# fuenshu/deap

Hardware: AMD Instinct MI355X
Metric: individual-generations/sec @pop=2^20 Rastrigin-1000D, 1-8 GPU; % HBM peak (higher is better)
Workload: dtype f64; 1 GPU; C3 Rastrigin-1000D fp64 eaSimple; pop_per_island=1048576, islands=1, islands_per_gpu=1, genes=1000, operators=selTournament(t=3) cxBlend mutGaussian cxpb=0.5 mutpb=0.2 indpb=0.05, parallelism=islands1

## Files before the change

deap_amd/csrc/capi.hip:

```cpp
#include <stdarg.h>
#include <stdio.h>

#include "common.hpp"
#include "evals.hpp"

namespace dm {

int zig_make_tables(double* t) {
    const double R = 3.6541528853610088, V = 0.00492867323399;
    double* x = t;
    double* f = t + (ZIG_N + 1);
    x[0] = V / std::exp(-0.5 * R * R);
    x[1] = R;
    for (int i = 2; i < ZIG_N; ++i)
        x[i] = std::sqrt(-2.0 * std::log(V / x[i - 1] + std::exp(-0.5 * x[i - 1] * x[i - 1])));
    x[ZIG_N] = 0.0;
    for (int i = 0; i <= ZIG_N; ++i) f[i] = std::exp(-0.5 * x[i] * x[i]);
    return DM_OK;
}

static thread_local char g_err[1024] = "";

void set_error(const char* fmt, ...) {
    va_list ap;
// ... 391 lines not shown
using namespace dm;

extern "C" {

const char* dm_last_error(void) { return dm::g_err; }
const char* dm_version(void) { return "deapmi 0.1 gfx950"; }

static int env_int(const char* name, int dflt) {
    const char* v = std::getenv(name);
    return v ? atoi(v) : dflt;
}

static void read_knobs(dm_knobs& kn) {
    kn.disable_pipe = std::getenv("DM_DISABLE_PIPE") != nullptr;
    kn.bits_plan = std::getenv("DM_BITS_PLAN") != nullptr;
    kn.bits_nokeys = std::getenv("DM_BITS_NOKEYS") != nullptr;
    kn.lex_full = std::getenv("DM_LEX_FULL") != nullptr;
    kn.lex_no32 = std::getenv("DM_LEX_NO32") != nullptr;
    kn.pipe_label_rounds = std::max(0, std::min(8, env_int("DM_PIPE_LABEL_ROUNDS", 2)));
    kn.selbest_fullsort = std::getenv("DM_SELBEST_FULLSORT") != nullptr;
    kn.pipe_bpc = std::max(0, env_int("DM_PIPE_BPC", 0));
    kn.pipe_noorder = std::getenv("DM_PIPE_NOORDER") != nullptr;
    kn.pipe_key_fitter = std::getenv("DM_PIPE_KEY_FITTER") != nullptr;
}

int dm_ctx_reload_knobs(dm_ctx* ctx) {
    DM_CHECK_ARG(ctx != nullptr, "null ctx");
    read_knobs(ctx->knobs);
    return DM_OK;
}

int dm_ctx_create(int device, void* hip_stream, dm_ctx** out) {
    DM_CHECK_ARG(out != nullptr, "null out");
    DM_HIP(hipSetDevice(device));
    dm_ctx* c = new dm_ctx();
    c->device = device;
    c->stream = (hipStream_t)hip_stream;
    read_knobs(c->knobs);
    int cus = 0;
    if (hipDeviceGetAttribute(&cus, hipDeviceAttributeMultiprocessorCount, device) == hipSuccess &&
        cus > 0)
        c->num_cus = cus;
    double tab[2 * (ZIG_N + 1)];
    zig_make_tables(tab);
    if (hipMalloc(&c->zig, sizeof(tab)) != hipSuccess ||
        hipMemcpy(c->zig, tab, sizeof(tab), hipMemcpyHostToDevice) != hipSuccess) {
// ... 279 lines not shown
```

deap_amd/csrc/common.hpp:

```cpp
#pragma once
#include <hip/hip_runtime.h>
#include <stdint.h>

#include <algorithm>
#include <cmath>
#include <cstdlib>
#include <string>
#include <vector>

#include "../../include/deapmi.h"

namespace dm {

void set_error(const char* fmt, ...);

#define DM_CHECK_ARG(cond, ...)                 \
    do {                                        \
        if (!(cond)) {                          \
            ::dm::set_error(__VA_ARGS__);       \
            return DM_ERR_INVALID;              \
        }                                       \
    } while (0)

#define DM_HIP(expr)                                                          \
// ... 3 lines not shown
            ::dm::set_error("HIP error %s at %s:%d: %s", hipGetErrorName(e_), \
                            __FILE__, __LINE__, #expr);                       \
            return DM_ERR_HIP;                                                \
        }                                                                     \
    } while (0)

#define DM_LAUNCH_CHECK() DM_HIP(hipGetLastError())

}

constexpr int kEvalSpread = 64, kEvalSpreadStride = 16;
constexpr int kEvalSpreadWords = (2 * kEvalSpread + 2) * kEvalSpreadStride;
struct dm_knobs {
    bool disable_pipe = false;
    bool bits_plan = false;
    bool bits_nokeys = false;
    bool lex_full = false;
    bool lex_no32 = false;
    int32_t pipe_label_rounds = 2;
    bool selbest_fullsort = false;
    int pipe_bpc = 0;
    bool pipe_noorder = false;
    bool pipe_key_fitter = false;
};

struct dm_ctx {
    static constexpr int kSlots = 5;
    int device = 0;
    hipStream_t stream = nullptr;
    void* scratch[kSlots] = {nullptr, nullptr, nullptr, nullptr, nullptr};
    size_t scratch_bytes[kSlots] = {0, 0, 0, 0, 0};
    void* pinned = nullptr;
    size_t pinned_bytes = 0;
    int num_cus = 256;
    int peel_hint = 4;
    int peel_trend = 0;
    int64_t peel_hint_U = 0, peel_hint_N = 0;
    double* zig = nullptr;
    long long* evals_spread = nullptr;
    std::vector<hipEvent_t> tev;
    int tev_used = 0;
    int timing_target = 0;
    dm_knobs knobs;
    uint64_t* plan_lab = nullptr;
    int64_t plan_lab_n = 0;
    uint32_t plan_epoch = 0;
// ... 183 lines not shown
```

deap_amd/csrc/generation.hip:

```cpp
#include "generation_pipe.hpp"
#include "sort.hpp"

namespace dm {

__global__ __launch_bounds__(256) void zero2_kernel(int32_t* __restrict__ a, int32_t* __restrict__ b,
                                                    int64_t n) {
    const int64_t n4 = n >> 2;
    const int64_t step = (int64_t)gridDim.x * blockDim.x;
    for (int64_t i = (int64_t)blockIdx.x * blockDim.x + threadIdx.x; i < n4; i += step) {
        reinterpret_cast<int4*>(a)[i] = make_int4(0, 0, 0, 0);
        if (b) reinterpret_cast<int4*>(b)[i] = make_int4(0, 0, 0, 0);
    }
    for (int64_t i = 4 * n4 + (int64_t)blockIdx.x * blockDim.x + threadIdx.x; i < n; i += step) {
        a[i] = 0;
        if (b) b[i] = 0;
    }
}

static int pick_group_float(int dim) {
    const int q = (dim + 3) / 4;
    if (q <= 4) return 4;
    if (q <= 16) return 16;
    return 64;
}
// ... 104 lines not shown
    a.sigma = var->sigma;
    a.mu_vec = var->mu_vec;
    a.sigma_vec = var->sigma_vec;
    a.flip_inv_log2 = (var->indpb > 0.0 && var->indpb < 1.0)
                          ? (float)(1.0 / std::log2(1.0 - var->indpb))
                          : 0.0f;
    a.eval_fn = ev->fn;
    a.w0 = ev->weights[0];
    a.ev = *ev;
    a.rng = Rng(rng);
    a.zig = ctx->zig;
    a.mode = mode;
    a.dec = d;
    a.nevals = nevals;

    const int ec = eval_class(ev->fn);
    const int64_t npairs = (children->n + 1) / 2;
    if (mode == DM_RNG_NATIVE && parents->gtype != DM_BITS && parents->dim > 64 &&
        parents->dim <= 65535 && (sel == DM_SEL_TOURNAMENT || sel == DM_SEL_RANDOM) &&
        ec != EC_MO && !ctx->knobs.disable_pipe) {
        const int nch = parents->dim <= 512 ? 2 : parents->dim <= 1024 ? 4 : 0;
        const bool ordered = !ctx->knobs.pipe_noorder && npairs >= 4096 &&
                             npairs < (1ll << (32 - PF_PAIR_SHIFT));
        const size_t pb = align_up((size_t)npairs * sizeof(PairPlan), 256);
        const size_t hb = align_up((size_t)(a.np + 1) * 4, 256);
        const size_t kb = align_up((size_t)npairs * 4, 256);
        char* w = (char*)scratch(ctx, ordered ? 2 * pb + 3 * hb + 4 * kb +
                                                    align_up(scan_temp_bytes(a.np), 256) : pb);
        if (!w) return DM_ERR_NOMEM;
        PairPlan* plans = (PairPlan*)w;
        const bool count = ec != EC_NONE && a.nevals;
        if (ordered) {
            PairPlan* sorted = (PairPlan*)(w + pb);
            int32_t* hist = (int32_t*)(w + 2 * pb);
            int32_t* start = (int32_t*)(w + 2 * pb + hb);
            int32_t* keys = (int32_t*)(w + 2 * pb + 2 * hb);
            int32_t* tick = (int32_t*)(w + 2 * pb + 2 * hb + kb);
            void* stemp = w + 2 * pb + 2 * hb + 2 * kb;
            const unsigned zg = (unsigned)std::min<int64_t>(2048, (a.np / 4 + 255) / 256 + 1);
            if (!ctx->knobs.pipe_key_fitter && ctx->knobs.pipe_label_rounds > 0) {
                uint32_t epoch = 0;
                uint64_t* lab64 = plan_labels(ctx, a.np, &epoch);
                if (!lab64) return DM_ERR_NOMEM;
                int2* pairs2 = (int2*)((char*)stemp + align_up(scan_temp_bytes(a.np), 256));
                launch_pair_plans(a, plans, count ? ctx->evals_spread : nullptr, ctx->stream,
                                  nullptr, nullptr, nullptr, lab64, epoch, pairs2, hist, a.np + 1);
                const int rounds = ctx->knobs.pipe_label_rounds;
                if (rounds > 2)
                    launch_plan_labels(pairs2, lab64, epoch, npairs, rounds - 2, ctx->stream);
                launch_plan_degree_keys(plans, pairs2, nullptr, lab64, epoch, rounds >= 2, keys,
                                        tick, hist, npairs, ctx->stream);
            } else if (!ctx->knobs.pipe_key_fitter) {
                int32_t* deg = (int32_t*)((char*)stemp + align_up(scan_temp_bytes(a.np), 256));
                zero2_kernel<<<zg, 256, 0, ctx->stream>>>(hist, deg, a.np);
                launch_pair_plans(a, plans, count ? ctx->evals_spread : nullptr, ctx->stream,
                                  nullptr, deg);
                launch_plan_degree_keys(plans, nullptr, deg, nullptr, 0, false, keys, tick, hist,
                                        npairs, ctx->stream);
            } else {
                zero2_kernel<<<zg, 256, 0, ctx->stream>>>(hist, nullptr, a.np);
                launch_pair_plans(a, plans, count ? ctx->evals_spread : nullptr, ctx->stream, keys,
                                  hist, tick);
            }
            int rc = exclusive_scan_i32(ctx->stream, hist, start, a.np, nullptr, stemp);
            if (rc) return rc;
            launch_plan_order(plans, keys, tick, start, sorted, npairs, ctx->stream);
            plans = sorted;
        } else {
            launch_pair_plans(a, plans, count ? ctx->evals_spread : nullptr, ctx->stream);
        }
        DM_LAUNCH_CHECK();
        PipeArgs q{};
        q.pgenes = a.pgenes;
        q.cgenes = a.cgenes;
        q.cwv = a.cwv;
        q.cvalid = a.cvalid;
        q.plans = plans;
        q.pwv = a.pwv;
        q.mu_vec = a.mu_vec;
        q.sigma_vec = a.sigma_vec;
        q.zig = a.zig;
        q.nevals = nullptr;
        q.nc = a.nc;
        q.pstride = a.pstride;
        q.cstride = a.cstride;
        q.dim = a.dim;
        q.nobj = a.nobj;
        q.rng = a.rng;
        q.thr_ind = a.thr_ind;
        q.alpha = a.alpha;
        q.mu = a.mu;
        q.sigma = a.sigma;
        q.w0 = a.w0;
        q.ev = a.ev;
        q.bpc = ctx->knobs.pipe_bpc;
        q.ordered = ordered ? 1 : 0;
        timing_begin(ctx);
        if (parents->gtype == DM_F64)
            launch_gen_pipe_f64(q, ec, a.cx, a.mut, nch, ctx->num_cus, ctx->stream);
        else
            launch_gen_pipe_f32(q, ec, a.cx, a.mut, nch, ctx->num_cus, ctx->stream);
        timing_end(ctx);
        DM_LAUNCH_CHECK();
        return DM_OK;
    }
    if (mode == DM_RNG_NATIVE && parents->gtype != DM_BITS && parents->dim <= 64 &&
        (sel == DM_SEL_TOURNAMENT || sel == DM_SEL_RANDOM) && !ctx->knobs.disable_pipe) {
        PairPlan* plans = (PairPlan*)scratch(ctx, align_up((size_t)npairs * sizeof(PairPlan), 256));
        if (!plans) return DM_ERR_NOMEM;
        const bool count = ec != EC_NONE && a.nevals;
        launch_pair_plans(a, plans, count ? ctx->evals_spread : nullptr, ctx->stream);
        DM_LAUNCH_CHECK();
        timing_begin(ctx);
        if (parents->gtype == DM_F64)
            launch_gen_rows_f64(a, plans, ec, ctx->num_cus, ctx->stream);
        else
            launch_gen_rows_f32(a, plans, ec, ctx->num_cus, ctx->stream);
        timing_end(ctx);
        DM_LAUNCH_CHECK();
// ... 64 lines not shown
```

deap_amd/csrc/generation_pipe.hpp:

```cpp
#pragma once
#include "generation.hpp"

namespace dm {

typedef __attribute__((address_space(4))) const uint32_t c4_u32;

#ifndef DM_RAST_ILP
#define DM_RAST_ILP 2
#endif

struct PairPlan {
    int32_t s0, s1;
    uint32_t cuts;
    uint32_t flags;
    double f0, f1;
};
static_assert(sizeof(PairPlan) == 32, "PairPlan layout");
enum : uint32_t { PF_CX = 1, PF_MUT0 = 2, PF_MUT1 = 4, PF_HAS1 = 8, PF_INV0 = 16, PF_INV1 = 32 };
constexpr int PF_PAIR_SHIFT = 8;

__device__ __forceinline__ PairPlan load_plan(const PairPlan* plans, int64_t p) {
    const c4_u32* q = (const c4_u32*)(const void*)(plans + p);
    uint32_t v[8];
#pragma unroll
    for (int i = 0; i < 8; ++i) v[i] = q[i];
    PairPlan r;
    r.s0 = (int32_t)v[0];
    r.s1 = (int32_t)v[1];
    r.cuts = v[2];
    r.flags = v[3];
    r.f0 = __hiloint2double((int)v[5], (int)v[4]);
    r.f1 = __hiloint2double((int)v[7], (int)v[6]);
    return r;
}

#ifndef DM_ZIG_SLOW_NOINLINE
#define DM_ZIG_SLOW_NOINLINE 1
#endif
#if DM_ZIG_SLOW_NOINLINE
__device__ __noinline__
#else
__device__ __forceinline__
// ... 141 lines not shown
                const double v = k == 0 ? x[0] : k == 1 ? x[1] : k == 2 ? x[2] : x[3];
                if (L::gene(c, lane, k) < dim) t += sum_term(ev.fn, v);
            }
            acc += t;
        }
    }
}

struct PipeArgs {
    const char* pgenes;
    char* cgenes;
    double* cwv;
    uint8_t* cvalid;
    const PairPlan* plans;
    const double* pwv;
    const double* mu_vec;
    const double* sigma_vec;
    const double* zig;
    int64_t* nevals;
    int64_t nc, pstride, cstride;
    int32_t dim, nobj;
    int32_t bpc;
    int32_t ordered;
    Rng rng;
    uint64_t thr_ind;
    double alpha, mu, sigma, w0;
    dm_eval ev;
};

#ifndef DM_PIPE_MINWAVES
#define DM_PIPE_MINWAVES 2
#endif

#ifndef DM_PIPE_ABLATE
#define DM_PIPE_ABLATE 0
#endif

#ifndef DM_PIPE_DEPTH
#define DM_PIPE_DEPTH 2
#endif

template <typename T, int NCH, int CX, int MUT, int EC,
          int DEPTH = sizeof(T) == 4 ? 2 * DM_PIPE_DEPTH : DM_PIPE_DEPTH>
__global__ __launch_bounds__(256, DM_PIPE_MINWAVES) void gen_pipe_kernel(PipeArgs a) {
    typedef ChunkLayout<T> L;
    constexpr int D = NCH == 0 ? DEPTH : NCH < DEPTH ? NCH : DEPTH;
    static_assert(NCH % D == 0, "ring depth must divide the chunk count");
    __shared__ double szig[ZIG_N + 1];
    __shared__ double2 cstab[64];
    if (MUT == DM_MUT_GAUSSIAN)
        for (int i = threadIdx.x; i <= ZIG_N; i += blockDim.x) szig[i] = a.zig[i];
    if (EC == EC_RAST && threadIdx.x < 64) {
        double sn, cn;
        sincospi((double)threadIdx.x / 32.0, &sn, &cn);
        cstab[threadIdx.x] = make_double2(cn, sn);
    }
    if (MUT == DM_MUT_GAUSSIAN || EC == EC_RAST) __syncthreads();
    const int lane = threadIdx.x & 63;
    const int64_t npairs = (a.nc + 1) / 2;
    const int64_t nw = ((int64_t)gridDim.x * blockDim.x) >> 6;
    const int64_t wid = ((int64_t)blockIdx.x * blockDim.x + threadIdx.x) >> 6;
    int64_t j, jend, jstep;
    if (a.ordered) {
        const int64_t wpb = blockDim.x >> 6;
        const int64_t per = ((npairs + gridDim.x - 1) / gridDim.x + wpb - 1) / wpb * wpb;
        j = (int64_t)blockIdx.x * per + (threadIdx.x >> 6);
        jend = std::min<int64_t>(npairs, (int64_t)blockIdx.x * per + per);
        jstep = wpb;
    } else {
        j = wid;
        jend = npairs;
        jstep = nw;
    }
    if (j >= jend) return;
    int64_t evals = 0;
    const int dim = a.dim;
    const int nchr = NCH > 0 ? NCH : ((dim + 255) / 256 + D - 1) / D * D;
    const double gamma_scale = 1.0 + 2.0 * a.alpha;

    PairPlan pl = load_plan(a.plans, j);
    PairPlan nx = load_plan(a.plans, j + jstep < jend ? j + jstep : j);
    typename L::Raw y0[D], y1[D];
#pragma unroll
    for (int ch = 0; ch < D; ++ch) {
        L::load(a.pgenes + (int64_t)pl.s0 * a.pstride, ch, lane, dim, y0[ch]);
        L::load(a.pgenes + (int64_t)pl.s1 * a.pstride, ch, lane, dim, y1[ch]);
    }
    for (; j < jend; j += jstep) {
        const bool more = j + jstep < jend;
        const int64_t j2 = j + 2 * jstep;
        const PairPlan nn = load_plan(a.plans, j2 < jend ? j2 : j);
        const int64_t p = a.ordered ? (int64_t)(pl.flags >> PF_PAIR_SHIFT) : j;
        const int64_t c0 = 2 * p, c1 = 2 * p + 1;
        const uint32_t fl = pl.flags;
        const bool cx = fl & PF_CX, mut0 = fl & PF_MUT0, mut1 = fl & PF_MUT1;
        const bool has1 = fl & PF_HAS1, inv0 = fl & PF_INV0, inv1 = fl & PF_INV1;
        const int cp1 = (int)(pl.cuts & 0xFFFFu), cp2 = (int)(pl.cuts >> 16);
        char* w0 = a.cgenes + c0 * a.cstride;
        char* w1 = a.cgenes + c1 * a.cstride;
        const char* r0 = a.pgenes + (int64_t)pl.s0 * a.pstride;
        const char* r1 = a.pgenes + (int64_t)pl.s1 * a.pstride;
        const char* n0 = a.pgenes + (int64_t)nx.s0 * a.pstride;
        const char* n1 = a.pgenes + (int64_t)nx.s1 * a.pstride;
        double acc0 = 0.0, acc1 = 0.0, carry0 = 0.0, carry1 = 0.0;
        auto chunk = [&](const int ch, const int sl) {
            double x0[4], x1[4];
            L::unpack(y0[sl], x0);
            L::unpack(y1[sl], x1);
            {
                const int ca = ch + D;
                if (ca < nchr) {
                    L::load(r0, ca, lane, dim, y0[sl]);
                    L::load(r1, ca, lane, dim, y1[sl]);
                } else if (more) {
                    L::load(n0, ca - nchr, lane, dim, y0[sl]);
                    L::load(n1, ca - nchr, lane, dim, y1[sl]);
                }
            }
            const uint32_t slot = (uint32_t)((ch << 6) + lane);
            if (CX == DM_CX_BLEND && cx) {
                const u32x4 u = (DM_PIPE_ABLATE & 2) ? u32x4{1u << 31, 1u << 31, 1u << 31, 1u << 31}
                                                     : a.rng(ST_BLEND, (uint32_t)p, slot);
                const uint32_t us[4] = {u.x, u.y, u.z, u.w};
#pragma unroll
                for (int k = 0; k < 4; ++k) {
                    const double gm = gamma_scale * u01_32(us[k]) - a.alpha;
                    const double v1 = x0[k], v2 = x1[k];
                    x0[k] = (1.0 - gm) * v1 + gm * v2;
                    x1[k] = gm * v1 + (1.0 - gm) * v2;
                }
            } else if (CX == DM_CX_TWOPOINT && cx) {
#pragma unroll
                for (int k = 0; k < 4; ++k) {
                    const int gk = L::gene(ch, lane, k);
                    if (gk >= cp1 && gk < cp2) {
                        const double tt = x0[k];
                        x0[k] = x1[k];
                        x1[k] = tt;
                    }
// ... 10 lines not shown
                uint32_t keep = 0;
#pragma unroll
                for (int k = 0; k < 4; ++k) keep |= (L::gene(ch, lane, k) < dim ? 1u : 0u) << k;
                uint32_t bits = 0;
                if (mut0) {
                    const u32x4 w = a.rng(ST_MASK, (uint32_t)c0, slot);
                    bits |= ((uint64_t)w.x < a.thr_ind ? 1u : 0u) | ((uint64_t)w.y < a.thr_ind ? 2u : 0u) |
                            ((uint64_t)w.z < a.thr_ind ? 4u : 0u) | ((uint64_t)w.w < a.thr_ind ? 8u : 0u);
                }
                if (mut1) {
                    const u32x4 w = a.rng(ST_MASK, (uint32_t)c1, slot);
                    bits |= (((uint64_t)w.x < a.thr_ind ? 1u : 0u) | ((uint64_t)w.y < a.thr_ind ? 2u : 0u) |
                             ((uint64_t)w.z < a.thr_ind ? 4u : 0u) | ((uint64_t)w.w < a.thr_ind ? 8u : 0u))
                            << 4;
                }
                bits &= keep | (keep << 4);
#pragma unroll 1
                while (bits) {
                    const int b = __builtin_ctz(bits);
                    bits &= bits - 1;
                    const int j = b & 3;
                    const int gi = L::gene(ch, lane, j);
                    const double nrm =
                        zig_normal_lds(szig, a.zig, a.rng, (uint32_t)(c0 + (b >> 2)), (uint32_t)gi);
                    const double m = a.mu_vec ? a.mu_vec[gi] : a.mu;
                    const double s = a.sigma_vec ? a.sigma_vec[gi] : a.sigma;
                    const double gv = m + nrm * s;
                    if (b < 4) {
                        x0[0] = j == 0 ? x0[0] + gv : x0[0];
                        x0[1] = j == 1 ? x0[1] + gv : x0[1];
                        x0[2] = j == 2 ? x0[2] + gv : x0[2];
                        x0[3] = j == 3 ? x0[3] + gv : x0[3];
                    } else {
                        x1[0] = j == 0 ? x1[0] + gv : x1[0];
                        x1[1] = j == 1 ? x1[1] + gv : x1[1];
                        x1[2] = j == 2 ? x1[2] + gv : x1[2];
                        x1[3] = j == 3 ? x1[3] + gv : x1[3];
                    }
                }
            }
            L::store_nt(w0, ch, lane, dim, x0);
            if (has1) L::store_nt(w1, ch, lane, dim, x1);
            if constexpr (sizeof(T) == 4) {
#pragma unroll
                for (int k = 0; k < 4; ++k) {
                    x0[k] = (double)(float)x0[k];
                    x1[k] = (double)(float)x1[k];
// ... 31 lines not shown
                a.cwv[c0] = pl.f0;
                if (has1) a.cwv[c1] = pl.f1;
            } else {
                const int m = a.nobj;
                for (int o = 0; o < m; ++o) {
                    a.cwv[c0 * m + o] = a.pwv[(int64_t)pl.s0 * m + o];
                    if (has1) a.cwv[c1 * m + o] = a.pwv[(int64_t)pl.s1 * m + o];
                }
            }
            a.cvalid[c0] = inv0 ? 0 : 1;
            if (has1) a.cvalid[c1] = inv1 ? 0 : 1;
        }
        pl = nx;
        nx = nn;
    }
    if (a.nevals && EC != EC_NONE) {
        int64_t tot = evals;
#pragma unroll
        for (int o = 32; o > 0; o >>= 1) tot += __shfl_xor(tot, o, 64);
        if (lane == 0 && tot) atomicAdd((unsigned long long*)a.nevals, (unsigned long long)tot);
    }
}

inline dim3 pipe_grid(int num_cus, int64_t npairs, int bpc, bool ordered) {
    const int occ = bpc > 0 ? bpc : ordered ? 32 : 64;
    const int64_t blocks = std::min<int64_t>((npairs + 3) / 4, (int64_t)num_cus * occ);
    return dim3((unsigned)std::max<int64_t>(blocks, 1));
}
template <typename T, int NCH, int CX, int MUT, int EC>
void launch_pipe_k(const PipeArgs& a, int num_cus, hipStream_t s) {
    auto kern = gen_pipe_kernel<T, NCH, CX, MUT, EC>;
    kern<<<pipe_grid(num_cus, (a.nc + 1) / 2, a.bpc, a.ordered != 0), 256, 0, s>>>(a);
}
template <typename T, int NCH, int CX, int MUT>
void launch_pipe_e(const PipeArgs& a, int ec, int num_cus, hipStream_t s) {
    if (ec == EC_RAST)
        launch_pipe_k<T, NCH, CX, MUT, EC_RAST>(a, num_cus, s);
    else if (ec == EC_ROSEN)
        launch_pipe_k<T, NCH, CX, MUT, EC_ROSEN>(a, num_cus, s);
    else if (ec_single(ec))
        launch_pipe_k<T, NCH, CX, MUT, EC_SUM>(a, num_cus, s);
    else
        launch_pipe_k<T, NCH, CX, MUT, EC_NONE>(a, num_cus, s);
}
template <typename T, int NCH>
void launch_pipe_ops(const PipeArgs& a, int ec, int cx, int mut, int num_cus, hipStream_t s) {
    const bool mg = mut == DM_MUT_GAUSSIAN;
    switch (cx) {
        case DM_CX_BLEND:
            mg ? launch_pipe_e<T, NCH, DM_CX_BLEND, DM_MUT_GAUSSIAN>(a, ec, num_cus, s)
               : launch_pipe_e<T, NCH, DM_CX_BLEND, DM_MUT_NONE>(a, ec, num_cus, s);
            break;
        case DM_CX_TWOPOINT:
            mg ? launch_pipe_e<T, NCH, DM_CX_TWOPOINT, DM_MUT_GAUSSIAN>(a, ec, num_cus, s)
               : launch_pipe_e<T, NCH, DM_CX_TWOPOINT, DM_MUT_NONE>(a, ec, num_cus, s);
            break;
        default:
            mg ? launch_pipe_e<T, NCH, DM_CX_NONE, DM_MUT_GAUSSIAN>(a, ec, num_cus, s)
               : launch_pipe_e<T, NCH, DM_CX_NONE, DM_MUT_NONE>(a, ec, num_cus, s);
    }
}

void launch_pair_plans(const GenArgs& a, PairPlan* plans, long long* count_evals, hipStream_t s,
                       int32_t* keys = nullptr, int32_t* hist = nullptr,
                       int32_t* tick = nullptr, uint64_t* lab64 = nullptr, uint32_t epoch = 0,
                       int2* pairs2 = nullptr, int32_t* zero = nullptr, int64_t nzero = 0);
void launch_plan_order(const PairPlan* plans, const int32_t* keys, const int32_t* tick,
                       const int32_t* start, PairPlan* ordered, int64_t npairs, hipStream_t s);
void launch_plan_degree_keys(const PairPlan* plans, const int2* pairs2, const int32_t* deg,
                             const uint64_t* lab64, uint32_t epoch, bool jump, int32_t* keys,
                             int32_t* tick, int32_t* hist2, int64_t npairs, hipStream_t s);
void launch_plan_labels(const int2* pairs2, uint64_t* lab64, uint32_t epoch, int64_t npairs,
                        int rounds, hipStream_t s);
void launch_gen_bits_fused(const GenArgs& a, bool eval, long long* spread, hipStream_t s);
void launch_fit_keys(const GenArgs& a, int16_t* keys, hipStream_t s);
void launch_gen_pipe_f64(const PipeArgs& a, int ec, int cx, int mut, int nch, int num_cus,
                         hipStream_t s);
void launch_gen_pipe_f32(const PipeArgs& a, int ec, int cx, int mut, int nch, int num_cus,
                         hipStream_t s);
void launch_gen_rows_f64(const GenArgs& a, const PairPlan* plans, int ec, int num_cus,
                         hipStream_t s);
void launch_gen_rows_f32(const GenArgs& a, const PairPlan* plans, int ec, int num_cus,
                         hipStream_t s);
void launch_gen_pipe_long(const PipeArgs& a, bool f64, int ec, int cx, int mut, int num_cus,
                          hipStream_t s);
void launch_gen_bits_pipe(const GenArgs& a, const PairPlan* plans, bool eval, int num_cus,
                          hipStream_t s);

}
// ... 1 lines not shown
```

deap_amd/csrc/generation_pipe_f64.hip:

```cpp
#include "generation_pipe.hpp"

namespace dm {

__device__ __forceinline__ int32_t lab_of(const uint64_t* lab64, int32_t r, uint32_t epoch) {
    const uint64_t u = lab64[r];
    return (uint32_t)(u >> 32) == epoch ? min(INT32_MAX - (int32_t)(uint32_t)u, r) : r;
}
#ifndef DM_PLAN_ABLATE
#define DM_PLAN_ABLATE 0
#endif
__device__ __forceinline__ void lab_lower(uint64_t* lab64, int32_t r, int32_t m, uint32_t epoch) {
    if (DM_PLAN_ABLATE & 1) return;
    atomicMax((unsigned long long*)(lab64 + r),
              ((unsigned long long)epoch << 32) | (uint32_t)(INT32_MAX - m));
}

template <int MF>
__device__ __forceinline__ uint32_t plan_one(const GenArgs& a, PairPlan* __restrict__ plans,
                                             int64_t p, int32_t* __restrict__ keys,
                                             int32_t* __restrict__ hist,
                                             int32_t* __restrict__ tick,
                                             uint64_t* __restrict__ lab64, uint32_t epoch,
                                             int2* __restrict__ pairs2) {
    const int64_t c0 = 2 * p, c1 = 2 * p + 1;
    const bool has1 = c1 < a.nc;
    const int m = a.nobj;
    const uint32_t np = (uint32_t)a.np;
    int32_t s[2];
    constexpr int TM = MF == 1 ? 8 : 4;
    bool fast = a.sel == DM_SEL_TOURNAMENT && (MF == 1 ? m == 1 : (m >= 2 && m <= MF)) &&
                a.tournsize >= 1 && a.tournsize <= TM;
    double fw[2] = {0.0, 0.0};
    uint8_t vw[2] = {1, 1};
    if (fast && MF > 1) {
        const int t = a.tournsize;
        int32_t kk[2][TM];
        double ff[2][TM][MF];
#pragma unroll
        for (int h = 0; h < 2; ++h) {
            const uint32_t c = (uint32_t)(h ? c1 : c0);
            u32x4 w{};
#pragma unroll
            for (int j = 0; j < TM; ++j) {
                if (j < t && (h == 0 || has1)) {
                    if (!(j & 1)) w = a.rng(ST_SEL, c, (uint32_t)(j >> 1));
                    kk[h][j] = (int32_t)((j & 1) ? bounded64(w.z, w.w, np) : bounded64(w.x, w.y, np));
// ... 128 lines not shown
    } else {
        if (!cx && !(fl & PF_MUT0)) vw[0] = a.pvalid[s[0]];
        if (has1 && !cx && !(fl & PF_MUT1)) vw[1] = a.pvalid[s[1]];
        if (!has1) {
            vw[1] = vw[0];
            fw[1] = fw[0];
        }
    }
    if (cx || (fl & PF_MUT0) || !vw[0]) fl |= PF_INV0;
    if (has1 && (cx || (fl & PF_MUT1) || !vw[1])) fl |= PF_INV1;
    PairPlan pl;
    pl.s0 = s[0];
    pl.s1 = s[1];
    pl.cuts = cuts;
    pl.flags = fl;
    pl.f0 = fw[0];
    pl.f1 = fw[1];
    plans[p] = pl;
    if (keys && tick) {
        const int32_t key = pl.f1 > pl.f0 ? s[1] : s[0];
        keys[p] = key;
        tick[p] = atomicAdd(hist + key, 1);
    } else if (lab64) {
        if (pairs2) pairs2[p] = make_int2(s[0], s[1]);
        if (has1 && s[0] != s[1]) lab_lower(lab64, max(s[0], s[1]), min(s[0], s[1]), epoch);
    } else if (hist) {
        atomicAdd(hist + s[0], 1);
        if (has1) atomicAdd(hist + s[1], 1);
    }
    return fl;
}

template <int MF>
__global__ __launch_bounds__(256) void pair_plan_kernel(GenArgs a, PairPlan* __restrict__ plans,
                                                        long long* __restrict__ count_evals,
                                                        int32_t* __restrict__ keys,
                                                        int32_t* __restrict__ hist,
                                                        int32_t* __restrict__ tick,
                                                        uint64_t* __restrict__ lab64,
                                                        uint32_t epoch,
                                                        int2* __restrict__ pairs2,
                                                        int32_t* __restrict__ zero, int64_t nzero) {
    const int64_t p = (int64_t)blockIdx.x * blockDim.x + threadIdx.x;
    const int64_t npairs = (a.nc + 1) / 2;
    if (zero)
        for (int64_t i = p; i < nzero; i += (int64_t)gridDim.x * blockDim.x) zero[i] = 0;
    if (count_evals) {
        __shared__ int32_t wave_evals[4];
        uint32_t fl = 0;
        if (p < npairs) fl = plan_one<MF>(a, plans, p, keys, hist, tick, lab64, epoch, pairs2);
        const int32_t cnt = __popcll(__ballot((fl & PF_INV0) != 0)) +
                            __popcll(__ballot((fl & PF_INV1) != 0));
        if ((threadIdx.x & 63) == 0) wave_evals[threadIdx.x >> 6] = cnt;
        __syncthreads();
        if (threadIdx.x == 0)
            evals_fold(count_evals, a.nevals,
                       (long long)wave_evals[0] + wave_evals[1] + wave_evals[2] + wave_evals[3]);
        return;
    }
    if (p < npairs) plan_one<MF>(a, plans, p, keys, hist, tick, lab64, epoch, pairs2);
}

void launch_pair_plans(const GenArgs& a, PairPlan* plans, long long* count_evals, hipStream_t s,
                       int32_t* keys, int32_t* hist, int32_t* tick, uint64_t* lab64,
                       uint32_t epoch, int2* pairs2, int32_t* zero, int64_t nzero) {
    const int64_t npairs = (a.nc + 1) / 2;
    const dim3 grid((unsigned)((npairs + 255) / 256));
    if (a.nobj >= 2 && a.nobj <= 3)
        pair_plan_kernel<3><<<grid, 256, 0, s>>>(a, plans, count_evals, keys, hist, tick, lab64, epoch,
                                                 pairs2, zero, nzero);
    else
        pair_plan_kernel<1><<<grid, 256, 0, s>>>(a, plans, count_evals, keys, hist, tick, lab64, epoch,
                                                 pairs2, zero, nzero);
}

__global__ __launch_bounds__(256) void plan_order_kernel(const PairPlan* __restrict__ plans,
                                                         const int32_t* __restrict__ keys,
                                                         const int32_t* __restrict__ tick,
                                                         const int32_t* __restrict__ start,
                                                         PairPlan* __restrict__ ordered,
                                                         int64_t npairs) {
    const int64_t p = (int64_t)blockIdx.x * blockDim.x + threadIdx.x;
    if (p >= npairs) return;
    PairPlan pl = plans[p];
    pl.flags |= (uint32_t)p << PF_PAIR_SHIFT;
    ordered[start[keys[p]] + tick[p]] = pl;
}

__global__ __launch_bounds__(256) void plan_degree_key_kernel(const PairPlan* __restrict__ plans,
                                                              const int2* __restrict__ pairs2,
                                                              const int32_t* __restrict__ deg,
                                                              const uint64_t* __restrict__ lab64,
                                                              uint32_t epoch, int jump,
                                                              int32_t* __restrict__ keys,
                                                              int32_t* __restrict__ tick,
                                                              int32_t* __restrict__ hist2,
// ... 6 lines not shown
    if (lab64) {
        const int32_t l0 = lab_of(lab64, s0, epoch), l1 = lab_of(lab64, s1, epoch);
        bin = min(l0, l1);
        if (jump) bin = min(bin, min(lab_of(lab64, l0, epoch), lab_of(lab64, l1, epoch)));
    } else {
        bin = deg[s1] > deg[s0] ? s1 : s0;
    }
    keys[p] = bin;
    tick[p] = atomicAdd(hist2 + bin, 1);
}
void launch_plan_degree_keys(const PairPlan* plans, const int2* pairs2, const int32_t* deg,
                             const uint64_t* lab64, uint32_t epoch, bool jump, int32_t* keys,
                             int32_t* tick, int32_t* hist2, int64_t npairs, hipStream_t s) {
    plan_degree_key_kernel<<<dim3((unsigned)((npairs + 255) / 256)), 256, 0, s>>>(
        plans, pairs2, deg, lab64, epoch, jump ? 1 : 0, keys, tick, hist2, npairs);
}

__global__ __launch_bounds__(256) void plan_label_kernel(const int2* __restrict__ pairs2,
                                                         uint64_t* __restrict__ lab64,
                                                         uint32_t epoch, int64_t npairs) {
    const int64_t p = (int64_t)blockIdx.x * blockDim.x + threadIdx.x;
    if (p >= npairs) return;
    const int2 pr = pairs2[p];
    const int32_t s0 = pr.x, s1 = pr.y;
    const int32_t l0 = lab_of(lab64, s0, epoch), l1 = lab_of(lab64, s1, epoch);
    const int32_t m = min(l0, l1);
    if (m < l0) lab_lower(lab64, s0, m, epoch);
    if (m < l1) lab_lower(lab64, s1, m, epoch);
}
void launch_plan_labels(const int2* pairs2, uint64_t* lab64, uint32_t epoch, int64_t npairs,
                        int rounds, hipStream_t s) {
    for (int r = 0; r < rounds; ++r)
        plan_label_kernel<<<dim3((unsigned)((npairs + 255) / 256)), 256, 0, s>>>(pairs2, lab64,
                                                                                 epoch, npairs);
}

void launch_plan_order(const PairPlan* plans, const int32_t* keys, const int32_t* tick,
                       const int32_t* start, PairPlan* ordered, int64_t npairs, hipStream_t s) {
    plan_order_kernel<<<dim3((unsigned)((npairs + 255) / 256)), 256, 0, s>>>(plans, keys, tick,
                                                                            start, ordered, npairs);
}

void launch_gen_pipe_f64(const PipeArgs& a, int ec, int cx, int mut, int nch, int num_cus,
                         hipStream_t s) {
    if (nch == 0)
        launch_gen_pipe_long(a, true, ec, cx, mut, num_cus, s);
    else if (nch <= 2)
        launch_pipe_ops<double, 2>(a, ec, cx, mut, num_cus, s);
    else
        launch_pipe_ops<double, 4>(a, ec, cx, mut, num_cus, s);
}

}
```

tools_gpu/ab_inproc.py:

```python
import ctypes
import os
import sys

import torch

sys.path.insert(0, ".")
from deap_amd import _lib, algorithms, base, benchmarks, tools
from deap_amd.ops import RandomStream

cfg, var, values = sys.argv[1], sys.argv[2], sys.argv[3:]
rounds, G = int(os.environ.get("AB_ROUNDS", "6")), int(os.environ.get("AB_GENS", "8"))
tb = base.Toolbox()
if cfg == "c2":
    dim, gt, w, lo, hi = 4096, "bits", (1.0,), 0, 1
    tb.register("evaluate", benchmarks.onemax)
    tb.register("mate", tools.cxTwoPoint)
    tb.register("mutate", tools.mutFlipBit, indpb=0.05)
else:
    dim, gt, w, lo, hi = 1000, "f64", (-1.0,), -5.12, 5.12
    tb.register("evaluate", benchmarks.rastrigin)
    tb.register("mate", tools.cxBlend, alpha=0.5)
    tb.register("mutate", tools.mutGaussian, mu=0, sigma=1.0, indpb=0.05)
tb.register("select", tools.selTournament, tournsize=3)
n = 1 << 20
st = RandomStream(1234)
pop = tools.initPopulation(n=n, dim=dim, low=lo, high=hi, gtype=gt, weights=w, stream=st)
tb.evaluate(pop)
off = pop.like(n, capacity=n)
step = algorithms.GenerationStep(pop, tb, 0.5, 0.2)
nev = torch.zeros(1, dtype=torch.int64, device=pop.device)
ctx = pop.ctx.bind()
for _ in range(3):
    step.step(pop, off, st, ctypes.c_void_p(nev.data_ptr()))
    pop.swap_storage(off)
torch.cuda.synchronize()
res = {v: [] for v in values}
for r in range(rounds):
    for v in values:
        if v == "unset":
            os.environ.pop(var, None)
        else:
            os.environ[var] = v
        _lib.call("dm_ctx_reload_knobs", ctx)
        _lib.call("dm_ctx_set_timing", ctx, G)
        for _ in range(G):
            step.step(pop, off, st, ctypes.c_void_p(nev.data_ptr()))
            pop.swap_storage(off)
        torch.cuda.synchronize()
        times = (ctypes.c_float * G)()
        cnt = ctypes.c_int32(0)
        _lib.call("dm_ctx_kernel_times", ctx, times, G, ctypes.byref(cnt))
        res[v].extend(times[:cnt.value])
_lib.call("dm_ctx_set_timing", ctx, 0)
for v in values:
    t = sorted(res[v])
    print("%s %s=%s: mean %.4f ms  median %.4f ms  (%d launches)" % (
        cfg, var, v, sum(t) / len(t), t[len(t) // 2], len(t)), flush=True)
```

Baseline: 366.4 million individual-generations/sec.

## Add opt-in regrouping of uncrossed children by parent row for read reuse

Adds an optional plan ordering that splits uncrossed pairs into single children, bins them by parent row, and interleaves them with crossed pairs ordered by label, so concurrent waves share parent reads. The pipe kernel learns to skip the second parent load when both rows match, and gains a selectable block size of 256, 512 or 1024 threads. Both the regroup mode and the larger block size sit behind environment knobs that default off, so the default path only picks up the duplicate-load skip. That skip adds branches in the hot loop.

```diff
diff --git a/deap_amd/csrc/capi.hip b/deap_amd/csrc/capi.hip
--- a/deap_amd/csrc/capi.hip
+++ b/deap_amd/csrc/capi.hip
@@ -437,6 +437,9 @@
     kn.pipe_bpc = std::max(0, env_int("DM_PIPE_BPC", 0));
     kn.pipe_noorder = std::getenv("DM_PIPE_NOORDER") != nullptr;
     kn.pipe_key_fitter = std::getenv("DM_PIPE_KEY_FITTER") != nullptr;
+    kn.pipe_regroup = env_int("DM_PIPE_REGROUP", 0) != 0;
+    const int wpb_threads = env_int("DM_PIPE_WPB", 256);
+    kn.pipe_wpb = wpb_threads == 1024 ? 16 : wpb_threads == 512 ? 8 : 4;
 }
 
 int dm_ctx_reload_knobs(dm_ctx* ctx) {
diff --git a/deap_amd/csrc/common.hpp b/deap_amd/csrc/common.hpp
--- a/deap_amd/csrc/common.hpp
+++ b/deap_amd/csrc/common.hpp
@@ -49,6 +49,8 @@
     int pipe_bpc = 0;
     bool pipe_noorder = false;
     bool pipe_key_fitter = false;
+    bool pipe_regroup = false;
+    int pipe_wpb = 4;
 };
 
 struct dm_ctx {
diff --git a/deap_amd/csrc/generation.hip b/deap_amd/csrc/generation.hip
--- a/deap_amd/csrc/generation.hip
+++ b/deap_amd/csrc/generation.hip
@@ -150,11 +150,15 @@
         const int nch = parents->dim <= 512 ? 2 : parents->dim <= 1024 ? 4 : 0;
         const bool ordered = !ctx->knobs.pipe_noorder && npairs >= 4096 &&
                              npairs < (1ll << (32 - PF_PAIR_SHIFT));
+        const bool regroup = ordered && ctx->knobs.pipe_regroup && !ctx->knobs.pipe_key_fitter &&
+                             ctx->knobs.pipe_label_rounds > 0 &&
+                             a.nc <= (1ll << (32 - PF_PAIR_SHIFT));
+        const int64_t nbins = regroup ? 2 * a.np + 1 : a.np;
         const size_t pb = align_up((size_t)npairs * sizeof(PairPlan), 256);
-        const size_t hb = align_up((size_t)(a.np + 1) * 4, 256);
+        const size_t hb = align_up((size_t)(nbins + 1) * 4, 256);
         const size_t kb = align_up((size_t)npairs * 4, 256);
         char* w = (char*)scratch(ctx, ordered ? 2 * pb + 3 * hb + 4 * kb +
-                                                    align_up(scan_temp_bytes(a.np), 256) : pb);
+                                                    align_up(scan_temp_bytes(nbins), 256) : pb);
         if (!w) return DM_ERR_NOMEM;
         PairPlan* plans = (PairPlan*)w;
         const bool count = ec != EC_NONE && a.nevals;
@@ -170,14 +174,19 @@
                 uint32_t epoch = 0;
                 uint64_t* lab64 = plan_labels(ctx, a.np, &epoch);
                 if (!lab64) return DM_ERR_NOMEM;
-                int2* pairs2 = (int2*)((char*)stemp + align_up(scan_temp_bytes(a.np), 256));
+                int2* pairs2 = (int2*)((char*)stemp + align_up(scan_temp_bytes(nbins), 256));
                 launch_pair_plans(a, plans, count ? ctx->evals_spread : nullptr, ctx->stream,
-                                  nullptr, nullptr, nullptr, lab64, epoch, pairs2, hist, a.np + 1);
+                                  nullptr, nullptr, nullptr, lab64, epoch, pairs2, hist, nbins + 1,
+                                  regroup);
                 const int rounds = ctx->knobs.pipe_label_rounds;
                 if (rounds > 2)
                     launch_plan_labels(pairs2, lab64, epoch, npairs, rounds - 2, ctx->stream);
-                launch_plan_degree_keys(plans, pairs2, nullptr, lab64, epoch, rounds >= 2, keys,
-                                        tick, hist, npairs, ctx->stream);
+                if (regroup)
+                    launch_plan_regroup_keys(pairs2, lab64, epoch, rounds >= 2, keys, tick, hist,
+                                             a.np, npairs, a.nc, ctx->stream);
+                else
+                    launch_plan_degree_keys(plans, pairs2, nullptr, lab64, epoch, rounds >= 2, keys,
+                                            tick, hist, npairs, ctx->stream);
             } else if (!ctx->knobs.pipe_key_fitter) {
                 int32_t* deg = (int32_t*)((char*)stemp + align_up(scan_temp_bytes(a.np), 256));
                 zero2_kernel<<<zg, 256, 0, ctx->stream>>>(hist, deg, a.np);
@@ -190,9 +199,13 @@
                 launch_pair_plans(a, plans, count ? ctx->evals_spread : nullptr, ctx->stream, keys,
                                   hist, tick);
             }
-            int rc = exclusive_scan_i32(ctx->stream, hist, start, a.np, nullptr, stemp);
+            int rc = exclusive_scan_i32(ctx->stream, hist, start, nbins, nullptr, stemp);
             if (rc) return rc;
-            launch_plan_order(plans, keys, tick, start, sorted, npairs, ctx->stream);
+            if (regroup)
+                launch_plan_regroup_order(plans, keys, tick, start, sorted, a.np, npairs, a.nc,
+                                          ctx->knobs.pipe_wpb, ctx->stream);
+            else
+                launch_plan_order(plans, keys, tick, start, sorted, npairs, ctx->stream);
             plans = sorted;
         } else {
             launch_pair_plans(a, plans, count ? ctx->evals_spread : nullptr, ctx->stream);
@@ -222,7 +235,8 @@
         q.w0 = a.w0;
         q.ev = a.ev;
         q.bpc = ctx->knobs.pipe_bpc;
-        q.ordered = ordered ? 1 : 0;
+        q.ordered = regroup ? 2 : ordered ? 1 : 0;
+        q.wpb = ctx->knobs.pipe_wpb;
         timing_begin(ctx);
         if (parents->gtype == DM_F64)
             launch_gen_pipe_f64(q, ec, a.cx, a.mut, nch, ctx->num_cus, ctx->stream);
diff --git a/deap_amd/csrc/generation_pipe.hpp b/deap_amd/csrc/generation_pipe.hpp
--- a/deap_amd/csrc/generation_pipe.hpp
+++ b/deap_amd/csrc/generation_pipe.hpp
@@ -18,6 +18,22 @@
 static_assert(sizeof(PairPlan) == 32, "PairPlan layout");
 enum : uint32_t { PF_CX = 1, PF_MUT0 = 2, PF_MUT1 = 4, PF_HAS1 = 8, PF_INV0 = 16, PF_INV1 = 32 };
 constexpr int PF_PAIR_SHIFT = 8;
+
+struct RegroupShape {
+    int64_t U, C, G, Uf, Cf, Nf;
+    __host__ __device__ RegroupShape(int64_t S, int64_t nc, int64_t g)
+        : U((S + 1) >> 1), C((nc - S) >> 1), G(g), Uf(U / g), Cf(C / g), Nf(U / g + C / g) {}
+    __host__ __device__ int64_t single_slot(int64_t i) const {
+        const int64_t a = i / G;
+        if (a >= Uf) return Nf * G + (i - Uf * G);
+        return (((a + 1) * Nf + Uf - 1) / Uf - 1) * G + i % G;
+    }
+    __host__ __device__ int64_t crossed_slot(int64_t j) const {
+        const int64_t c = j / G;
+        if (c >= Cf) return Nf * G + (U - Uf * G) + (j - Cf * G);
+        return (c * Nf / Cf) * G + j % G;
+    }
+};
 
 __device__ __forceinline__ PairPlan load_plan(const PairPlan* plans, int64_t p) {
     const c4_u32* q = (const c4_u32*)(const void*)(plans + p);
@@ -205,6 +221,7 @@
     int32_t dim, nobj;
     int32_t bpc;
     int32_t ordered;
+    int32_t wpb;
     Rng rng;
     uint64_t thr_ind;
     double alpha, mu, sigma, w0;
@@ -223,9 +240,9 @@
 #define DM_PIPE_DEPTH 2
 #endif
 
-template <typename T, int NCH, int CX, int MUT, int EC,
+template <typename T, int NCH, int CX, int MUT, int EC, int NT = 256,
           int DEPTH = sizeof(T) == 4 ? 2 * DM_PIPE_DEPTH : DM_PIPE_DEPTH>
-__global__ __launch_bounds__(256, DM_PIPE_MINWAVES) void gen_pipe_kernel(PipeArgs a) {
+__global__ __launch_bounds__(NT, DM_PIPE_MINWAVES) void gen_pipe_kernel(PipeArgs a) {
     typedef ChunkLayout<T> L;
     constexpr int D = NCH == 0 ? DEPTH : NCH < DEPTH ? NCH : DEPTH;
     static_assert(NCH % D == 0, "ring depth must divide the chunk count");
@@ -267,15 +284,17 @@
 #pragma unroll
     for (int ch = 0; ch < D; ++ch) {
         L::load(a.pgenes + (int64_t)pl.s0 * a.pstride, ch, lane, dim, y0[ch]);
-        L::load(a.pgenes + (int64_t)pl.s1 * a.pstride, ch, lane, dim, y1[ch]);
+        if (pl.s1 != pl.s0) L::load(a.pgenes + (int64_t)pl.s1 * a.pstride, ch, lane, dim, y1[ch]);
     }
     for (; j < jend; j += jstep) {
         const bool more = j + jstep < jend;
         const int64_t j2 = j + 2 * jstep;
         const PairPlan nn = load_plan(a.plans, j2 < jend ? j2 : j);
         const int64_t p = a.ordered ? (int64_t)(pl.flags >> PF_PAIR_SHIFT) : j;
-        const int64_t c0 = 2 * p, c1 = 2 * p + 1;
-        const uint32_t fl = pl.flags;
+        const bool sg = a.ordered == 2 && !(pl.flags & PF_CX);
+        const int64_t c0 = sg ? p : 2 * p;
+        const int64_t c1 = sg ? (int64_t)(pl.cuts >> PF_PAIR_SHIFT) : 2 * p + 1;
+        const uint32_t fl = sg ? pl.flags | (pl.cuts & (PF_MUT1 | PF_INV1)) : pl.flags;
         const bool cx = fl & PF_CX, mut0 = fl & PF_MUT0, mut1 = fl & PF_MUT1;
         const bool has1 = fl & PF_HAS1, inv0 = fl & PF_INV0, inv1 = fl & PF_INV1;
         const int cp1 = (int)(pl.cuts & 0xFFFFu), cp2 = (int)(pl.cuts >> 16);
@@ -286,18 +305,22 @@
         const char* n0 = a.pgenes + (int64_t)nx.s0 * a.pstride;
         const char* n1 = a.pgenes + (int64_t)nx.s1 * a.pstride;
         double acc0 = 0.0, acc1 = 0.0, carry0 = 0.0, carry1 = 0.0;
+        const bool same = pl.s1 == pl.s0, nsame = nx.s1 == nx.s0;
         auto chunk = [&](const int ch, const int sl) {
             double x0[4], x1[4];
             L::unpack(y0[sl], x0);
-            L::unpack(y1[sl], x1);
+            if (same)
+                L::unpack(y0[sl], x1);
+            else
+                L::unpack(y1[sl], x1);
             {
                 const int ca = ch + D;
                 if (ca < nchr) {
                     L::load(r0, ca, lane, dim, y0[sl]);
-                    L::load(r1, ca, lane, dim, y1[sl]);
+                    if (!same) L::load(r1, ca, lane, dim, y1[sl]);
                 } else if (more) {
                     L::load(n0, ca - nchr, lane, dim, y0[sl]);
-                    L::load(n1, ca - nchr, lane, dim, y1[sl]);
+                    if (!nsame) L::load(n1, ca - nchr, lane, dim, y1[sl]);
                 }
             }
             const uint32_t slot = (uint32_t)((ch << 6) + lane);
@@ -354,7 +377,7 @@
                     const int j = b & 3;
                     const int gi = L::gene(ch, lane, j);
                     const double nrm =
-                        zig_normal_lds(szig, a.zig, a.rng, (uint32_t)(c0 + (b >> 2)), (uint32_t)gi);
+                        zig_normal_lds(szig, a.zig, a.rng, (uint32_t)(b < 4 ? c0 : c1), (uint32_t)gi);
                     const double m = a.mu_vec ? a.mu_vec[gi] : a.mu;
                     const double s = a.sigma_vec ? a.sigma_vec[gi] : a.sigma;
                     const double gv = m + nrm * s;
@@ -432,15 +455,21 @@
     }
 }
 
-inline dim3 pipe_grid(int num_cus, int64_t npairs, int bpc, bool ordered) {
-    const int occ = bpc > 0 ? bpc : ordered ? 32 : 64;
-    const int64_t blocks = std::min<int64_t>((npairs + 3) / 4, (int64_t)num_cus * occ);
+inline dim3 pipe_grid(int num_cus, int64_t npairs, int bpc, bool ordered, int wpb = 4) {
+    const int occ = std::max(1, (bpc > 0 ? bpc : ordered ? 32 : 64) * 4 / wpb);
+    const int64_t blocks = std::min<int64_t>((npairs + wpb - 1) / wpb, (int64_t)num_cus * occ);
     return dim3((unsigned)std::max<int64_t>(blocks, 1));
 }
 template <typename T, int NCH, int CX, int MUT, int EC>
 void launch_pipe_k(const PipeArgs& a, int num_cus, hipStream_t s) {
-    auto kern = gen_pipe_kernel<T, NCH, CX, MUT, EC>;
-    kern<<<pipe_grid(num_cus, (a.nc + 1) / 2, a.bpc, a.ordered != 0), 256, 0, s>>>(a);
+    const int wpb = a.wpb == 8 || a.wpb == 16 ? a.wpb : 4;
+    const dim3 grid = pipe_grid(num_cus, (a.nc + 1) / 2, a.bpc, a.ordered != 0, wpb);
+    if (wpb == 16)
+        gen_pipe_kernel<T, NCH, CX, MUT, EC, 1024><<<grid, 1024, 0, s>>>(a);
+    else if (wpb == 8)
+        gen_pipe_kernel<T, NCH, CX, MUT, EC, 512><<<grid, 512, 0, s>>>(a);
+    else
+        gen_pipe_kernel<T, NCH, CX, MUT, EC, 256><<<grid, 256, 0, s>>>(a);
 }
 template <typename T, int NCH, int CX, int MUT>
 void launch_pipe_e(const PipeArgs& a, int ec, int num_cus, hipStream_t s) {
@@ -474,7 +503,14 @@
 void launch_pair_plans(const GenArgs& a, PairPlan* plans, long long* count_evals, hipStream_t s,
                        int32_t* keys = nullptr, int32_t* hist = nullptr,
                        int32_t* tick = nullptr, uint64_t* lab64 = nullptr, uint32_t epoch = 0,
-                       int2* pairs2 = nullptr, int32_t* zero = nullptr, int64_t nzero = 0);
+                       int2* pairs2 = nullptr, int32_t* zero = nullptr, int64_t nzero = 0,
+                       bool regroup = false);
+void launch_plan_regroup_keys(const int2* pairs2, const uint64_t* lab64, uint32_t epoch, bool jump,
+                              int32_t* keys, int32_t* tick, int32_t* hist, int64_t np,
+                              int64_t npairs, int64_t nc, hipStream_t s);
+void launch_plan_regroup_order(const PairPlan* plans, const int32_t* keys, const int32_t* tick,
+                               const int32_t* start, PairPlan* ordered, int64_t np, int64_t npairs,
+                               int64_t nc, int group, hipStream_t s);
 void launch_plan_order(const PairPlan* plans, const int32_t* keys, const int32_t* tick,
                        const int32_t* start, PairPlan* ordered, int64_t npairs, hipStream_t s);
 void launch_plan_degree_keys(const PairPlan* plans, const int2* pairs2, const int32_t* deg,
diff --git a/deap_amd/csrc/generation_pipe_f64.hip b/deap_amd/csrc/generation_pipe_f64.hip
--- a/deap_amd/csrc/generation_pipe_f64.hip
+++ b/deap_amd/csrc/generation_pipe_f64.hip
@@ -21,7 +21,7 @@
                                              int32_t* __restrict__ hist,
                                              int32_t* __restrict__ tick,
                                              uint64_t* __restrict__ lab64, uint32_t epoch,
-                                             int2* __restrict__ pairs2) {
+                                             int2* __restrict__ pairs2, bool regroup) {
     const int64_t c0 = 2 * p, c1 = 2 * p + 1;
     const bool has1 = c1 < a.nc;
     const int m = a.nobj;
@@ -196,8 +196,10 @@
         keys[p] = key;
         tick[p] = atomicAdd(hist + key, 1);
     } else if (lab64) {
-        if (pairs2) pairs2[p] = make_int2(s[0], s[1]);
-        if (has1 && s[0] != s[1]) lab_lower(lab64, max(s[0], s[1]), min(s[0], s[1]), epoch);
+        const bool single = regroup && !cx;
+        if (pairs2) pairs2[p] = make_int2(single ? ~s[0] : s[0], s[1]);
+        if (has1 && s[0] != s[1] && !single)
+            lab_lower(lab64, max(s[0], s[1]), min(s[0], s[1]), epoch);
     } else if (hist) {
         atomicAdd(hist + s[0], 1);
         if (has1) atomicAdd(hist + s[1], 1);
@@ -214,7 +216,8 @@
                                                         uint64_t* __restrict__ lab64,
                                                         uint32_t epoch,
                                                         int2* __restrict__ pairs2,
-                                                        int32_t* __restrict__ zero, int64_t nzero) {
+                                                        int32_t* __restrict__ zero, int64_t nzero,
+                                                        bool regroup) {
     const int64_t p = (int64_t)blockIdx.x * blockDim.x + threadIdx.x;
     const int64_t npairs = (a.nc + 1) / 2;
     if (zero)
@@ -222,7 +225,7 @@
     if (count_evals) {
         __shared__ int32_t wave_evals[4];
         uint32_t fl = 0;
-        if (p < npairs) fl = plan_one<MF>(a, plans, p, keys, hist, tick, lab64, epoch, pairs2);
+        if (p < npairs) fl = plan_one<MF>(a, plans, p, keys, hist, tick, lab64, epoch, pairs2, regroup);
         const int32_t cnt = __popcll(__ballot((fl & PF_INV0) != 0)) +
                             __popcll(__ballot((fl & PF_INV1) != 0));
         if ((threadIdx.x & 63) == 0) wave_evals[threadIdx.x >> 6] = cnt;
@@ -232,20 +235,20 @@
                        (long long)wave_evals[0] + wave_evals[1] + wave_evals[2] + wave_evals[3]);
         return;
     }
-    if (p < npairs) plan_one<MF>(a, plans, p, keys, hist, tick, lab64, epoch, pairs2);
+    if (p < npairs) plan_one<MF>(a, plans, p, keys, hist, tick, lab64, epoch, pairs2, regroup);
 }
 
 void launch_pair_plans(const GenArgs& a, PairPlan* plans, long long* count_evals, hipStream_t s,
                        int32_t* keys, int32_t* hist, int32_t* tick, uint64_t* lab64,
-                       uint32_t epoch, int2* pairs2, int32_t* zero, int64_t nzero) {
+                       uint32_t epoch, int2* pairs2, int32_t* zero, int64_t nzero, bool regroup) {
     const int64_t npairs = (a.nc + 1) / 2;
     const dim3 grid((unsigned)((npairs + 255) / 256));
     if (a.nobj >= 2 && a.nobj <= 3)
         pair_plan_kernel<3><<<grid, 256, 0, s>>>(a, plans, count_evals, keys, hist, tick, lab64, epoch,
-                                                 pairs2, zero, nzero);
+                                                 pairs2, zero, nzero, regroup);
     else
         pair_plan_kernel<1><<<grid, 256, 0, s>>>(a, plans, count_evals, keys, hist, tick, lab64, epoch,
-                                                 pairs2, zero, nzero);
+                                                 pairs2, zero, nzero, regroup);
 }
 
 __global__ __launch_bounds__(256) void plan_order_kernel(const PairPlan* __restrict__ plans,
@@ -298,6 +301,7 @@
     const int64_t p = (int64_t)blockIdx.x * blockDim.x + threadIdx.x;
     if (p >= npairs) return;
     const int2 pr = pairs2[p];
+    if (pr.x < 0) return;
     const int32_t s0 = pr.x, s1 = pr.y;
     const int32_t l0 = lab_of(lab64, s0, epoch), l1 = lab_of(lab64, s1, epoch);
     const int32_t m = min(l0, l1);
@@ -315,6 +319,87 @@
                        const int32_t* start, PairPlan* ordered, int64_t npairs, hipStream_t s) {
     plan_order_kernel<<<dim3((unsigned)((npairs + 255) / 256)), 256, 0, s>>>(plans, keys, tick,
                                                                             start, ordered, npairs);
+}
+
+__global__ __launch_bounds__(256) void plan_regroup_key_kernel(const int2* __restrict__ pairs2,
+                                                               const uint64_t* __restrict__ lab64,
+                                                               uint32_t epoch, int jump,
+                                                               int32_t* __restrict__ keys,
+                                                               int32_t* __restrict__ tick,
+                                                               int32_t* __restrict__ hist,
+                                                               int64_t np, int64_t npairs,
+                                                               int64_t nc) {
+    const int64_t p = (int64_t)blockIdx.x * blockDim.x + threadIdx.x;
+    if (p >= npairs) return;
+    const int2 pr = pairs2[p];
+    if (pr.x < 0) {
+        tick[p] = atomicAdd(hist + ~pr.x, 1);
+        if (2 * p + 1 < nc) keys[p] = atomicAdd(hist + pr.y, 1);
+        return;
+    }
+    const int32_t l0 = lab_of(lab64, pr.x, epoch), l1 = lab_of(lab64, pr.y, epoch);
+    int32_t bin = min(l0, l1);
+    if (jump) bin = min(bin, min(lab_of(lab64, l0, epoch), lab_of(lab64, l1, epoch)));
+    keys[p] = bin;
+    tick[p] = atomicAdd(hist + np + bin, 1);
+}
+void launch_plan_regroup_keys(const int2* pairs2, const uint64_t* lab64, uint32_t epoch, bool jump,
+                              int32_t* keys, int32_t* tick, int32_t* hist, int64_t np,
+                              int64_t npairs, int64_t nc, hipStream_t s) {
+    plan_regroup_key_kernel<<<dim3((unsigned)((npairs + 255) / 256)), 256, 0, s>>>(
+        pairs2, lab64, epoch, jump ? 1 : 0, keys, tick, hist, np, npairs, nc);
+}
+
+__device__ __forceinline__ void place_single(PairPlan* __restrict__ ordered,
+                                             const RegroupShape& sh, int64_t k, int64_t S,
+                                             int32_t row, double f, int64_t child, bool mut,
+                                             bool inv) {
+    PairPlan* q = ordered + sh.single_slot(k >> 1);
+    const uint32_t idx = (uint32_t)child << PF_PAIR_SHIFT;
+    if (!(k & 1)) {
+        const bool has1 = k + 1 < S;
+        q->s0 = row;
+        q->flags = idx | (mut ? PF_MUT0 : 0u) | (inv ? PF_INV0 : 0u) | (has1 ? PF_HAS1 : 0u);
+        q->f0 = f;
+        if (!has1) {
+            q->s1 = row;
+            q->cuts = idx;
+            q->f1 = f;
+        }
+    } else {
+        q->s1 = row;
+        q->cuts = idx | (mut ? PF_MUT1 : 0u) | (inv ? PF_INV1 : 0u);
+        q->f1 = f;
+    }
+}
+__global__ __launch_bounds__(256) void plan_regroup_order_kernel(const PairPlan* __restrict__ plans,
+                                                                 const int32_t* __restrict__ keys,
+                                                                 const int32_t* __restrict__ tick,
+                                                                 const int32_t* __restrict__ start,
+                                                                 PairPlan* __restrict__ ordered,
+                                                                 int64_t np, int64_t npairs,
+                                                                 int64_t nc, int group) {
+    const int64_t p = (int64_t)blockIdx.x * blockDim.x + threadIdx.x;
+    if (p >= npairs) return;
+    PairPlan pl = plans[p];
+    const int64_t S = start[np];
+    const RegroupShape sh(S, nc, group);
+    if (pl.flags & PF_CX) {
+        pl.flags |= (uint32_t)p << PF_PAIR_SHIFT;
+        ordered[sh.crossed_slot((int64_t)start[np + keys[p]] - S + tick[p])] = pl;
+        return;
+    }
+    place_single(ordered, sh, (int64_t)start[pl.s0] + tick[p], S, pl.s0, pl.f0, 2 * p,
+                 pl.flags & PF_MUT0, pl.flags & PF_INV0);
+    if (pl.flags & PF_HAS1)
+        place_single(ordered, sh, (int64_t)start[pl.s1] + keys[p], S, pl.s1, pl.f1, 2 * p + 1,
+                     pl.flags & PF_MUT1, pl.flags & PF_INV1);
+}
+void launch_plan_regroup_order(const PairPlan* plans, const int32_t* keys, const int32_t* tick,
+                               const int32_t* start, PairPlan* ordered, int64_t np, int64_t npairs,
+                               int64_t nc, int group, hipStream_t s) {
+    plan_regroup_order_kernel<<<dim3((unsigned)((npairs + 255) / 256)), 256, 0, s>>>(
+        plans, keys, tick, start, ordered, np, npairs, nc, group);
 }
 
 void launch_gen_pipe_f64(const PipeArgs& a, int ec, int cx, int mut, int nch, int num_cus,
diff --git a/tools_gpu/ab_inproc.py b/tools_gpu/ab_inproc.py
--- a/tools_gpu/ab_inproc.py
+++ b/tools_gpu/ab_inproc.py
@@ -1,6 +1,7 @@
 import ctypes
 import os
 import sys
+import time
 
 import torch
 
@@ -18,6 +19,10 @@
     tb.register("mutate", tools.mutFlipBit, indpb=0.05)
 else:
     dim, gt, w, lo, hi = 1000, "f64", (-1.0,), -5.12, 5.12
+    if cfg == "c3f32":
+        gt = "f32"
+    elif cfg == "c3d2000":
+        dim = 2000
     tb.register("evaluate", benchmarks.rastrigin)
     tb.register("mate", tools.cxBlend, alpha=0.5)
     tb.register("mutate", tools.mutGaussian, mu=0, sigma=1.0, indpb=0.05)
@@ -35,6 +40,8 @@
     pop.swap_storage(off)
 torch.cuda.synchronize()
 res = {v: [] for v in values}
+step_ms = {v: [] for v in values}
+kern_ms = {v: [] for v in values}
 for r in range(rounds):
     for v in values:
         if v == "unset":
@@ -43,16 +50,25 @@
             os.environ[var] = v
         _lib.call("dm_ctx_reload_knobs", ctx)
         _lib.call("dm_ctx_set_timing", ctx, G)
+        torch.cuda.synchronize()
+        t0 = time.perf_counter()
         for _ in range(G):
             step.step(pop, off, st, ctypes.c_void_p(nev.data_ptr()))
             pop.swap_storage(off)
         torch.cuda.synchronize()
+        step_ms[v].append((time.perf_counter() - t0) * 1e3 / G)
         times = (ctypes.c_float * G)()
         cnt = ctypes.c_int32(0)
         _lib.call("dm_ctx_kernel_times", ctx, times, G, ctypes.byref(cnt))
         res[v].extend(times[:cnt.value])
+        kern_ms[v].append(sum(times[:cnt.value]) / max(cnt.value, 1))
 _lib.call("dm_ctx_set_timing", ctx, 0)
 for v in values:
     t = sorted(res[v])
     print("%s %s=%s: mean %.4f ms  median %.4f ms  (%d launches)" % (
         cfg, var, v, sum(t) / len(t), t[len(t) // 2], len(t)), flush=True)
+for v in values:
+    print("%s %s=%s: step %.4f ms (rounds %.4f .. %.4f)  kernel per round %s  step per round %s" % (
+        cfg, var, v, sum(step_ms[v]) / rounds, min(step_ms[v]), max(step_ms[v]),
+        " ".join("%.4f" % x for x in kern_ms[v]), " ".join("%.4f" % x for x in step_ms[v])),
+        flush=True)
diff --git a/tools_gpu/plan_regroup_sim.py b/tools_gpu/plan_regroup_sim.py
--- /dev/null
+++ b/tools_gpu/plan_regroup_sim.py
@@ -0,0 +1,64 @@
+import sys
+
+import numpy as np
+
+lg = int(sys.argv[1]) if len(sys.argv) > 1 else 20
+cxpb = float(sys.argv[2]) if len(sys.argv) > 2 else 0.5
+n, t = 1 << lg, 3
+rng = np.random.default_rng(1)
+fit = rng.standard_normal(n)
+asp = rng.integers(0, n, size=(n, t))
+win = asp[np.arange(n), np.argmax(fit[asp], axis=1)]
+a, b = win[0::2], win[1::2]
+cx = rng.random(n // 2) < cxpb
+WINDOWS = (1, 2, 4, 8, 16, 64)
+
+
+def reads(r0, r1, w):
+    g = np.arange(len(r0), dtype=np.int64) // w
+    key = np.concatenate([g, g]) * n + np.concatenate([r0, r1])
+    return len(np.unique(key)) / n
+
+
+def label_order(a, b):
+    lab = np.arange(n)
+    np.minimum.at(lab, np.maximum(a, b), np.minimum(a, b))
+    l0, l1 = lab[a], lab[b]
+    bins = np.minimum(np.minimum(l0, l1), np.minimum(lab[l0], lab[l1]))
+    return np.argsort(bins, kind="stable")
+
+
+print("n = 2^%d, t = %d, cxpb = %g: distinct rows %.3f n, uncrossed pairs %.3f"
+      % (lg, t, cxpb, len(np.unique(win)) / n, 1 - cx.mean()))
+o = label_order(a, b)
+today = [reads(a[o], b[o], w) for w in WINDOWS]
+
+ac, bc = a[cx], b[cx]
+oc = label_order(ac, bc)
+crossed = [reads(ac[oc], bc[oc], w) for w in WINDOWS]
+
+s = np.sort(np.concatenate([a[~cx], b[~cx]]))
+if len(s) % 2:
+    s = np.append(s, s[-1])
+singles = [reads(s[0::2], s[1::2], w) for w in WINDOWS]
+same = float(np.mean(s[0::2] == s[1::2]))
+
+rows, cnt = np.unique(s, return_counts=True)
+fused = np.repeat(rows, cnt // 2)
+left = rows[cnt % 2 == 1]
+if len(left) % 2:
+    left = np.append(left, left[-1])
+f0, f1 = np.concatenate([fused, left[0::2]]), np.concatenate([fused, left[1::2]])
+of = np.argsort(f0, kind="stable")
+f0, f1 = f0[of], f1[of]
+fuse = [reads(f0, f1, w) for w in WINDOWS]
+
+print("window of plans      " + "".join("%8d" % w for w in WINDOWS))
+for name, row in (("label order", today),
+                  ("regrouped", [x + y for x, y in zip(singles, crossed)]),
+                  ("  singles", singles), ("  crossed", crossed),
+                  ("regrouped+fuse", [x + y for x, y in zip(fuse, crossed)]),
+                  ("  singles", fuse)):
+    print("%-21s" % name + "".join("%8.3f" % x for x in row))
+print("singles' plans with s0 == s1: %.3f (fused first: %.3f)"
+      % (same, float(np.mean(f0 == f1))))
```

Measured after the change: 370.4 million individual-generations/sec (median of 6 runs). 1.1% higher.
